# facebookresearch/brainmagick

Measured on AMD Instinct MI355X. Metric: segments/s, 208-ch x 360-sample SimpleConv + ClipLoss training step, higher is better.
Workload: dtype f32 (fp32-accurate: operands split into 2 scaled f16 planes, 3 MFMA products, fp32 accumulate; same parity tolerances as exact fp32, see DESIGN.md §2); 1 GPU; cfg2: gwilliams2022-shaped MEG C=208 T=360, F=120 features, 27 subjects, clip_conv SimpleConv (8985590 params) + ClipLoss + Adam; batch_per_gpu=256, global_batch=256, negatives=local, parallelism=dp1, comm=none, rccl_world=1, candidate_gather=none, distinct_batches=8

## Files before the change

brainmagick_amd/csrc/bm_common.h:

```cpp
#pragma once
#include <hip/hip_runtime.h>
#include <stdint.h>
#include <stdio.h>
#include <math.h>

typedef float f32x16 __attribute__((ext_vector_type(16)));
typedef float f32x4 __attribute__((ext_vector_type(4)));

#define BM_OK 0
#define BM_ERR_ARG 1001
#define BM_ERR_WORKSPACE 1002
#define BM_ERR_UNSUPPORTED 1003

extern thread_local char bm_err_buf[512];
int bm_set_error(int code, const char* fmt, ...);
int bm_check_launch(const char* what);

#define BM_REQUIRE(cond, ...)                                   \
    do {                                                        \
        if (!(cond)) return bm_set_error(BM_ERR_ARG, __VA_ARGS__); \
    } while (0)

static inline int cdiv(long a, long b) { return (int)((a + b - 1) / b); }
static inline bool prefer_big(int n) { return (long)cdiv(n, 128) * 128 <= (long)cdiv(n, 64) * 64; }
// ... 16 lines not shown
#else
    const unsigned t = (unsigned)(((unsigned long long)n * f.mul) >> 32);
#endif
    return f.shift == 0 ? n : (t + ((n - t) >> 1)) >> (f.shift - 1);
}
__host__ __device__ __forceinline__ int bm_floordiv(int a, int b) { return a >= 0 ? a / b : -((-a + b - 1) / b); }

#define BM_BKC 16
#define BM_WAVE 64

__device__ __forceinline__ int bm_xcd_remap(int id, int n) {
    const int q = n >> 3, r = n & 7;
    const int xcd = id & 7, slot = id >> 3;
    const int base = (xcd < r) ? xcd * (q + 1) : r * (q + 1) + (xcd - r) * q;
    return base + slot;
}

enum { BM_ACT_NONE = 0, BM_ACT_GELU = 1, BM_ACT_RELU = 2, BM_ACT_LEAKY = 3 };

__device__ __forceinline__ float bm_erff(float a) { return erff(a); }

__device__ __forceinline__ float bm_act(float z, int act, float leak) {
    if (act == BM_ACT_GELU) return 0.5f * z * (1.0f + bm_erff(z * 0.70710678118654752440f));
    if (act == BM_ACT_RELU) return !(z <= 0.f) ? z : 0.f;
    if (act == BM_ACT_LEAKY) return z > 0.f ? z : z * leak;
    return z;
}

__device__ __forceinline__ float bm_gelu_grad_fast(float z) {
    const float a = fabsf(z);
// ... 88 lines not shown
```

brainmagick_amd/csrc/core.hip:

```cpp
#include "bm_block.h"
#include <stdarg.h>
#include <stdlib.h>

thread_local char bm_err_buf[512] = {0};

int bm_set_error(int code, const char* fmt, ...) {
    va_list ap;
    va_start(ap, fmt);
    vsnprintf(bm_err_buf, sizeof(bm_err_buf), fmt, ap);
    va_end(ap);
    return code;
}

int bm_check_launch(const char* what) {
    hipError_t e = hipGetLastError();
    if (e != hipSuccess) return bm_set_error((int)e, "%s: launch failed: %s", what, hipGetErrorString(e));
    return BM_OK;
}

extern "C" const char* bm_last_error(void) { return bm_err_buf; }
extern "C" int bm_version(void) { return 117; }

extern "C" int bm_device_count(void) {
    int n = 0;
    hipError_t e = hipGetDeviceCount(&n);
    if (e != hipSuccess) { bm_set_error((int)e, "hipGetDeviceCount: %s", hipGetErrorString(e)); return -1; }
    return n;
}

#define FIN_THREADS 1024
#define FIN_WAVES (FIN_THREADS / 64)
__global__ __launch_bounds__(FIN_THREADS) void amax_finalize_kernel(const float* __restrict__ ws, int n,
                                                                    float* __restrict__ out) {
    __shared__ float sh[FIN_WAVES];
    bm_amax_fold<FIN_WAVES>(ws, n, out, sh);
}
// ... 38 lines not shown
```

brainmagick_amd/csrc/gemm_nt_h2w.hip:

```cpp
#include <cstdlib>
#include "gemm_nt_common.h"

typedef _Float16 f16x8 __attribute__((ext_vector_type(8)));
typedef _Float16 f16x4 __attribute__((ext_vector_type(4)));
typedef unsigned int u32x2 __attribute__((ext_vector_type(2)));

#define HG_K 32
#define HG_XQ (64 + 2)

struct GemmNTArgsH {
    const float* a; long a_sstride; long a_rstride;
    const float* x; long x_sstride; long x_rstride;
    const float* a_amax; const float* x_amax;
    const float* a_row_amax;
    float* part;
    int S, M, Cn, T, dil, nsplit;
    int tiles_m, tiles_c;
    const int* order; const int* seg;
};

__device__ __forceinline__ u32x4 hg_ld128(__amdgpu_buffer_rsrc_t rs, int voff, int soff) {
    return __builtin_amdgcn_raw_buffer_load_b128(rs, voff, soff, 0);
}
__device__ __forceinline__ unsigned hg_ld32(__amdgpu_buffer_rsrc_t rs, int voff) {
// ... 47 lines not shown
    else
        asm volatile("" :: "v"(r[0]), "v"(r[1]), "v"(r[2]), "v"(r[3]), "v"(r[4]), "v"(r[5]), "v"(r[6]), "v"(r[7]),
                     "v"(r[8]), "v"(r[9]), "v"(r[10]), "v"(r[11]));
}

#ifdef HG_TRACE
__device__ long long hg_trace_buf[64 * 4 * 8];
#define HG_T(I_) { __builtin_amdgcn_sched_barrier(0); tr[I_] = __builtin_readcyclecounter(); __builtin_amdgcn_sched_barrier(0); }
extern "C" int bm_debug_trace_read(long long* out) {
    return (int)hipMemcpyFromSymbol(out, HIP_SYMBOL(hg_trace_buf), sizeof(long long) * 64 * 4 * 8);
}
#else
#define HG_T(I_)
#endif

template <int KS, int MW, int NS, bool RS = false, bool TS = false, bool FL = false>
__global__ __launch_bounds__(256, 1) void gemm_nt_h2w_kernel(GemmNTArgsH a) {
    static_assert(!FL || RS, "the flat walk relies on the row-scaled A path (pieces inside or outside a row)");
    static_assert((MW == 5 && NS == 3) || (MW == 4 && NS == 2) || (MW == 4 && NS == 4),
                  "tile variants: 320 x 192, 256 x 128, 256 x 256");
    static_assert(!TS || (KS == 1 && !RS), "the transposed partial tile is the score contraction's");
    static_assert(KS == 1 || NS == 3, "3 taps use the 3 slots");
    constexpr int NA = 2 * MW;
    constexpr int NX = 2 * NS;
    constexpr int NP = NA + NX;
    constexpr int BM = 64 * MW;
    constexpr int BC = KS == 3 ? 64 : 64 * NS;
    constexpr int AQ = BM + 2;
    constexpr int ASLOTS = 4 * AQ;
    constexpr int PLANE = ASLOTS + NS * 4 * HG_XQ;
    constexpr int BUF = 2 * PLANE;
    constexpr int TN = MW * NS;
    constexpr int NXS = KS == 3 ? 3 : 1;
#ifdef HG_TRACE
    const long long t_kernel0 = __builtin_readcyclecounter();
    long long t_loop0 = t_kernel0, t_loop1 = t_kernel0;
#endif
    extern __shared__ __attribute__((aligned(16))) float smem[];
    u32x4* lds = reinterpret_cast<u32x4*>(smem);
    const int tid = threadIdx.x;
    const int lane = tid & 63;
    const int wave = __builtin_amdgcn_readfirstlane(tid >> 6);
    const int wm = wave >> 1, wc = wave & 1;
    const int nl = lane & 31, h = lane >> 5;

    int id = bm_xcd_remap(blockIdx.x, gridDim.x);
    const int tm = id % a.tiles_m; id /= a.tiles_m;
    const int tc = id % a.tiles_c; id /= a.tiles_c;
    const int split = id % a.nsplit;
    const int grp = id / a.nsplit;
    const int m0 = tm * BM, c0 = tc * BC;
    const int s_first = a.seg ? a.seg[grp] : 0;
    const int s_count = a.seg ? a.seg[grp + 1] - s_first : a.S;
#define HG_SEG(K_) (a.order ? a.order[s_first + (K_)] : s_first + (K_))

    const int cps = (a.T + HG_K - 1) / HG_K;
    const long nchunks = FL ? ((long)a.S * a.T + HG_K - 1) / HG_K : (long)s_count * cps;
    const long q_begin = nchunks * split / a.nsplit;
    const long q_end = nchunks * (split + 1) / a.nsplit;
    const int nst = (int)(q_end - q_begin);
    const int halo = KS == 3 ? a.dil : 0;
// ... 319 lines not shown
                }
            }
        }
    }
#ifdef HG_TRACE
    asm volatile("s_waitcnt vmcnt(0)" ::: "memory");
    if (blockIdx.x < 64 && lane == 0) {
        long long* o = hg_trace_buf + (blockIdx.x * 4 + wave) * 8;
        o[2] = t_loop0 - t_kernel0;
        o[3] = t_loop1 - t_loop0;
        o[6] = (long long)__builtin_readcyclecounter() - t_loop1;
    }
#endif
}

static int hg_family(int S, int G, int M, int Cn, int T, int KS, int dil, bool ordered) {
    if (KS != 3 && KS != 1) return 0;
    if ((G != 1 || ordered) && KS != 1) return 0;
    if (dil < 1 || dil > 32 || T < 2 * HG_K) return 0;
    if ((long)S * ((T + HG_K - 1) / HG_K) < 32L * G) return 0;
    const long work = (long)M * Cn;
    const long pad53 = (long)cdiv(M, 320) * 320 * cdiv(Cn, KS == 3 ? 64 : 192) * (KS == 3 ? 64 : 192);
    if (KS == 3) return pad53 * 4 <= work * 5 ? 1 : 0;
    const long pad42 = (long)cdiv(M, 256) * 256 * cdiv(Cn, 128) * 128;
    if (pad42 < pad53 && pad42 <= work * 2) return 2;
    return pad53 <= work * 2 ? 1 : 0;
}

extern "C" int bm_gemm_nt_h2_covers(int M, int Cn, int KS, int S, int T, int G, int dil, int ordered) {
    return hg_family(S, G, M, Cn, T, KS, dil, ordered != 0) ? 1 : 0;
// ... 1 lines not shown

extern "C" int bm_gemm_nt_h2_suggest_splits(int M, int Cn, int KS, int S, int T) {
    return bm_gemm_nt_h2_suggest_splits_grouped(M, Cn, KS, S, T, 1);
}
extern "C" int bm_gemm_nt_h2_suggest_splits_grouped(int M, int Cn, int KS, int S, int T, int G) {
    if (G < 1) G = 1;
    const int fam = hg_family(S, G, M, Cn, T, KS, 1, G > 1);
    const int tiles = (fam == 2 ? cdiv(M, 256) * cdiv(Cn, 128) : cdiv(M, 320) * cdiv(Cn, KS == 3 ? 64 : 192)) * G;
    const long chunks = (long)(S / G > 0 ? S / G : 1) * ((T + HG_K - 1) / HG_K);
    long want = 256 / tiles;
    if (want > chunks / 8) want = chunks / 8;
    if (want < 1) want = 1;
    return (int)want;
}

template <int KS, int MW, int NS, bool RS = false, bool TS = false, bool FL = false>
static int launch_gemm_nt_h2w(GemmNTArgsH g, hipStream_t stream, int ngroups = 1) {
    constexpr int PLANE = 4 * (64 * MW + 2) + NS * 4 * HG_XQ;
    const size_t lds = (size_t)2 * 2 * PLANE * 16;
    static bool attr_set = false;
    if (!attr_set) {
        hipError_t e = hipFuncSetAttribute(reinterpret_cast<const void*>(gemm_nt_h2w_kernel<KS, MW, NS, RS, TS, FL>),
                                           hipFuncAttributeMaxDynamicSharedMemorySize, (int)lds);
        if (e != hipSuccess) return bm_set_error((int)e, "gemm_nt_h2w: hipFuncSetAttribute: %s", hipGetErrorString(e));
        attr_set = true;
    }
    g.tiles_m = cdiv(g.M, 64 * MW);
    g.tiles_c = cdiv(g.Cn, KS == 3 ? 64 : 64 * NS);
    const long nblocks = (long)g.tiles_m * g.tiles_c * g.nsplit * ngroups;
    hipLaunchKernelGGL((gemm_nt_h2w_kernel<KS, MW, NS, RS, TS, FL>), dim3((unsigned)nblocks), dim3(256), lds, stream, g);
    return bm_check_launch("gemm_nt_h2w");
}

static int gemm_nt_h2_impl(const float* a, long a_sstride, long a_rstride, const float* a_amax, const float* a_row_amax,
                           const float* x, long x_sstride, long x_rstride, const float* x_amax, float* part, int S,
                           int M, int Cn, int T, int KS, int dil, int nsplit, void* stream,
                           const int* order = nullptr, const int* seg = nullptr, int G = 1) {
    BM_REQUIRE(a && x && part && a_amax && x_amax, "gemm_nt_h2: null pointer");
    BM_REQUIRE(M > 0 && Cn > 0 && T > 0 && nsplit > 0 && S >= 0, "gemm_nt_h2: bad dims");
    BM_REQUIRE(G >= 1 && (G == 1 || seg), "gemm_nt_h2: a grouped call needs seg[]");
    const bool grouped = seg != nullptr || order != nullptr;
    const int fam = hg_family(S, G, M, Cn, T, KS, dil, grouped);
    BM_REQUIRE(fam != 0, "gemm_nt_h2: shape not covered (M=%d Cn=%d T=%d KS=%d dil=%d)", M, Cn, T, KS, dil);
    if (((long)(M - 1) * a_rstride + T) * 4 >= 0x7f000000L || ((long)(Cn - 1) * x_rstride + T) * 4 >= 0x7f000000L)
        return bm_gemm_nt_x3(a, a_sstride, a_rstride, x, x_sstride, x_rstride, order, seg, part, S, G, M, Cn, T,
                             KS, dil, nsplit, stream);
    GemmNTArgsH g;
    g.a = a; g.a_sstride = a_sstride; g.a_rstride = a_rstride; g.a_amax = a_amax;
    g.x = x; g.x_sstride = x_sstride; g.x_rstride = x_rstride; g.x_amax = x_amax;
    g.a_row_amax = a_row_amax;
    g.part = part; g.S = S; g.M = M; g.Cn = Cn; g.T = T; g.dil = dil; g.nsplit = nsplit;
    g.order = order; g.seg = seg;
    hipStream_t s = (hipStream_t)stream;
    if (grouped) {
        if (fam == 2) return launch_gemm_nt_h2w<1, 4, 2>(g, s, G);
        return launch_gemm_nt_h2w<1, 5, 3>(g, s, G);
    }
    const bool rs = a_row_amax && fam == 1 && T % 4 == 0 && a_rstride % 4 == 0 && a_sstride % 4 == 0;
    const bool flat = rs && KS == 3 && T % HG_K != 0 && T >= 2 * HG_K && S > 1 &&
                      ((long)(S - 1) * a_sstride + (long)(M - 1) * a_rstride + T) * 4 < 0x7f000000L &&
                      ((long)(S - 1) * x_sstride + (long)(Cn - 1) * x_rstride + T) * 4 < 0x7f000000L &&
                      a_sstride >= T && x_sstride >= T && x_sstride % 4 == 0;
    if (flat) return launch_gemm_nt_h2w<3, 5, 3, true, false, true>(g, s);
    if (KS == 3) return rs ? launch_gemm_nt_h2w<3, 5, 3, true>(g, s) : launch_gemm_nt_h2w<3, 5, 3>(g, s);
    if (fam == 2) return launch_gemm_nt_h2w<1, 4, 2>(g, s);
    return rs ? launch_gemm_nt_h2w<1, 5, 3, true>(g, s) : launch_gemm_nt_h2w<1, 5, 3>(g, s);
}

extern "C" int bm_gemm_nt_h2(const float* a, long a_sstride, long a_rstride, const float* a_amax, const float* x,
                             long x_sstride, long x_rstride, const float* x_amax, float* part, int S, int M, int Cn,
                             int T, int KS, int dil, int nsplit, void* stream) {
    return gemm_nt_h2_impl(a, a_sstride, a_rstride, a_amax, nullptr, x, x_sstride, x_rstride, x_amax, part, S, M, Cn, T,
                           KS, dil, nsplit, stream);
}

extern "C" int bm_gemm_nt_h2_rows(const float* a, long a_sstride, long a_rstride, const float* a_amax,
                                  const float* a_row_amax, const float* x, long x_sstride, long x_rstride,
                                  const float* x_amax, float* part, int S, int M, int Cn, int T, int KS, int dil,
                                  int nsplit, void* stream) {
    return gemm_nt_h2_impl(a, a_sstride, a_rstride, a_amax, a_row_amax, x, x_sstride, x_rstride, x_amax, part, S, M, Cn,
                           T, KS, dil, nsplit, stream);
// ... 48 lines not shown
```

brainmagick_amd/csrc/pack.hip:

```cpp
#include "bm_common.h"

__global__ void pack_weights_kernel(const float* __restrict__ src, float* __restrict__ dst, int G,
                                    int M, int Cin, int KS, long sg, long sm, long sc, long sj,
                                    int flip, int Mpad, int nchunk, const float* alpha_ptr) {
    const long total = (long)G * nchunk * KS * BM_BKC * Mpad;
    const float alpha = alpha_ptr ? *alpha_ptr : 1.f;
    for (long i = (long)blockIdx.x * blockDim.x + threadIdx.x; i < total;
         i += (long)gridDim.x * blockDim.x) {
        long r = i;
        const int m = (int)(r % Mpad); r /= Mpad;
        const int cc = (int)(r % BM_BKC); r /= BM_BKC;
        const int j = (int)(r % KS); r /= KS;
        const int chunk = (int)(r % nchunk);
        const int g = (int)(r / nchunk);
        const int c = chunk * BM_BKC + cc;
        float v = 0.f;
        if (m < M && c < Cin) {
            const int jj = flip ? KS - 1 - j : j;
            v = alpha * src[g * sg + m * sm + c * sc + jj * sj];
        }
        dst[i] = v;
    }
}

// ... 78 lines not shown
        if (err) atomicExch(err, 1);
        v = 0;
    }
    out[i] = (int)v;
}

extern "C" int bm_index_to_i32(const long* idx, int B, int G, int* out, int* err_flag, void* stream) {
    BM_REQUIRE((idx && out) || B == 0, "index_to_i32: null pointer");
    BM_REQUIRE(B >= 0 && G > 0, "index_to_i32: bad dims B=%d G=%d", B, G);
    if (B == 0) return BM_OK;
    hipLaunchKernelGGL(index_to_i32_kernel, dim3((B + 255) / 256), dim3(256), 0, (hipStream_t)stream, idx, B,
                       G, out, err_flag);
    return bm_check_launch("index_to_i32");
}

__global__ void reduce_splits_kernel(const float* __restrict__ part, float* __restrict__ out, int G,
                                     int nsplit, int M, int Cn, int KS, long sg, long sm, long sc,
                                     long sj) {
    const long N = (long)Cn * KS;
    const long per = (long)M * N;
    const long total = (long)G * per;
    for (long i = (long)blockIdx.x * blockDim.x + threadIdx.x; i < total;
         i += (long)gridDim.x * blockDim.x) {
        const int g = (int)(i / per);
        const long r = i - (long)g * per;
        const int m = (int)(r / N);
        const int n = (int)(r - (long)m * N);
        const int c = n / KS, j = n - c * KS;
        const float* p = part + (long)g * nsplit * per + r;
        float s = 0.f;
        for (int k = 0; k < nsplit; ++k) s += p[(long)k * per];
        out[g * sg + m * sm + c * sc + j * sj] = s;
    }
}

__global__ void reduce_splits_vec4_kernel(const float* __restrict__ part, float* __restrict__ out, int G,
                                          int nsplit, int M, int Cn, int KS, long sg, long sm, long sc,
                                          long sj) {
    const long N = (long)Cn * KS;
    const long per = (long)M * N;
    const long total4 = (long)G * per / 4;
    for (long i4 = (long)blockIdx.x * blockDim.x + threadIdx.x; i4 < total4;
         i4 += (long)gridDim.x * blockDim.x) {
        const long i = i4 * 4;
        const int g = (int)(i / per);
        const long r = i - (long)g * per;
        const float* p = part + (long)g * nsplit * per + r;
        float4 s = make_float4(0.f, 0.f, 0.f, 0.f);
        int k = 0;
        for (; k + 8 <= nsplit; k += 8) {
            float4 v[8];
#pragma unroll
            for (int u = 0; u < 8; ++u) v[u] = *reinterpret_cast<const float4*>(p + (long)(k + u) * per);
#pragma unroll
            for (int u = 0; u < 8; ++u) { s.x += v[u].x; s.y += v[u].y; s.z += v[u].z; s.w += v[u].w; }
        }
        for (; k < nsplit; ++k) {
            const float4 v = *reinterpret_cast<const float4*>(p + (long)k * per);
            s.x += v.x; s.y += v.y; s.z += v.z; s.w += v.w;
        }
        const float sv[4] = {s.x, s.y, s.z, s.w};
#pragma unroll
        for (int e = 0; e < 4; ++e) {
            const long re = r + e;
            const int m = (int)(re / N);
            const int n = (int)(re - (long)m * N);
            const int c = n / KS, j = n - c * KS;
            out[g * sg + m * sm + c * sc + j * sj] = sv[e];
        }
    }
}

extern "C" int bm_reduce_splits(const float* part, float* out, int G, int nsplit, int M, int Cn,
                                int KS, long sg, long sm, long sc, long sj, void* stream) {
    BM_REQUIRE(part && out, "reduce_splits: null pointer");
    const long total = (long)G * M * Cn * KS;
    if (total <= 0) return BM_OK;
    const long per = (long)M * Cn * KS;
    if (per % 4 == 0 && ((uintptr_t)part % 16) == 0) {
        const long t4 = total / 4;
        const int blocks = (int)((t4 + 255) / 256 > 8192 ? 8192 : (t4 + 255) / 256);
        hipLaunchKernelGGL(reduce_splits_vec4_kernel, dim3(blocks), dim3(256), 0, (hipStream_t)stream, part,
                           out, G, nsplit, M, Cn, KS, sg, sm, sc, sj);
        return bm_check_launch("reduce_splits");
    }
    const int blocks = (int)((total + 255) / 256 > 8192 ? 8192 : (total + 255) / 256);
    hipLaunchKernelGGL(reduce_splits_kernel, dim3(blocks), dim3(256), 0, (hipStream_t)stream, part,
                       out, G, nsplit, M, Cn, KS, sg, sm, sc, sj);
    return bm_check_launch("reduce_splits");
}

__global__ void sum_over_batch_kernel(const float* __restrict__ x, float* __restrict__ out, int B,
                                      long n) {
    for (long i = (long)blockIdx.x * blockDim.x + threadIdx.x; i < n;
         i += (long)gridDim.x * blockDim.x) {
        float s = 0.f;
        for (int b = 0; b < B; ++b) s += x[(long)b * n + i];
        out[i] = s;
    }
}

extern "C" int bm_sum_over_batch(const float* x, float* out, int B, long n, void* stream) {
    BM_REQUIRE(x && out, "sum_over_batch: null pointer");
    if (n <= 0) return BM_OK;
// ... 6 lines not shown
```

brainmagick_amd/csrc/pack_h2.hip:

```cpp
#include "conv_h2_common.h"

extern "C" long bm_packed_weight_bytes_h2(int G, int M, int Cin, int KS) {
    const long mpad = bm_conv_h2_mpad(M);
    return (long)G * cdiv(Cin, 32) * KS * 2 * 4 * mpad * 8 * 2 + (long)G * mpad * 4;
}

struct PackH2Job {
    const float* src;
    unsigned short* dst;
    float* wscale;
    const float* alpha;
    long sg, sm, sc, sj;
    int M, Cin, KS, flip, Mpad, nchunk;
    int block0, nblocks;
};

#define PACK_ROWS 4

__device__ __forceinline__ void pack_h2_rows(const PackH2Job& jb, int block, float* tile, float* rs) {
    const float* __restrict__ src = jb.src;
    const int M = jb.M, Cin = jb.Cin, KS = jb.KS, Mpad = jb.Mpad, nchunk = jb.nchunk, flip = jb.flip;
    const long sg = jb.sg, sm = jb.sm, sc = jb.sc, sj = jb.sj;
    const int rows_per_group = Mpad / PACK_ROWS;
    const int g = block / rows_per_group, m0 = (block - g * rows_per_group) * PACK_ROWS;
// ... 52 lines not shown
        }
        const long stage = ((long)g * nchunk + chunk) * KS + j;
        unsigned short* out = jb.dst + stage * 2 * plane_stride + ((long)kg * Mpad + m0 + r) * 8;
        *reinterpret_cast<uint4*>(out) = *reinterpret_cast<const uint4*>(hi);
        *reinterpret_cast<uint4*>(out + plane_stride) = *reinterpret_cast<const uint4*>(lo);
    }
}

__global__ __launch_bounds__(256) void pack_weights_h2_kernel(PackH2Job jb) {
    extern __shared__ float pack_smem[];
    pack_h2_rows(jb, blockIdx.x, pack_smem + PACK_ROWS, pack_smem);
}

__global__ __launch_bounds__(256) void pack_weights_h2_batch_kernel(const PackH2Job* __restrict__ jobs, int njobs) {
    extern __shared__ float pack_smem[];
    int lo = 0, hi = njobs - 1;
    while (lo < hi) {
        const int mid = (lo + hi + 1) >> 1;
        if (jobs[mid].block0 <= (int)blockIdx.x) lo = mid; else hi = mid - 1;
    }
    const PackH2Job jb = jobs[lo];
    pack_h2_rows(jb, blockIdx.x - jb.block0, pack_smem + PACK_ROWS, pack_smem);
}

static int pack_h2_fill(PackH2Job& jb, const float* src, void* dst, int G, int M, int Cin, int KS, long sg, long sm,
                        long sc, long sj, int flip, const float* alpha_ptr) {
    BM_REQUIRE(src && dst, "pack_weights_h2: null pointer");
    BM_REQUIRE(G > 0 && M > 0 && Cin > 0 && KS > 0, "pack_weights_h2: bad dims");
    jb.Mpad = bm_conv_h2_mpad(M);
    jb.nchunk = cdiv(Cin, 32);
    const long f16_elems = (long)G * jb.nchunk * KS * 2 * 4 * jb.Mpad * 8;
    jb.src = src; jb.dst = (unsigned short*)dst;
    jb.wscale = reinterpret_cast<float*>(reinterpret_cast<char*>(dst) + f16_elems * 2);
    jb.alpha = alpha_ptr;
    jb.sg = sg; jb.sm = sm; jb.sc = sc; jb.sj = sj;
    jb.M = M; jb.Cin = Cin; jb.KS = KS; jb.flip = flip;
// ... 78 lines not shown
```

brainmagick_amd/functional.py:

```python

import torch

from . import hip_ops as H



ACT_CODES = {"none": H.ACT_NONE, "gelu": H.ACT_GELU, "relu": H.ACT_RELU, "leaky": H.ACT_LEAKY}


def _c(t: torch.Tensor) -> torch.Tensor:
    return t if t.is_contiguous() else t.contiguous()


_arange_cache = {}


def _arange_i32(n: int, device, repeat: int = 1) -> torch.Tensor:
    key = (n, repeat, device.type, device.index)
    t = _arange_cache.get(key)
    if t is None:
        if len(_arange_cache) > 64:
            _arange_cache.clear()
        t = torch.arange(n, dtype=torch.int32, device=device)
        if repeat != 1:
# ... 1 lines not shown
        if device.type == "cuda":
            torch.cuda.current_stream(device).synchronize()
        _arange_cache[key] = t
    return t


def _conv_weight_grads(dy, x, weight, KS, dil, transposed_weight):
    dst = H.grad_destination(weight)
    B, M, T = dy.shape
    Cin = x.shape[1]
    if transposed_weight:
        out = dst if dst is not None else torch.empty(weight.shape, device=dy.device, dtype=torch.float32)
        H.gemm_nt(x, dy, B, Cin, M, T, 1, 1, out=out.view(1, Cin, M, 1))
        return out.view(weight.shape) if dst is not None else out
    if dst is not None:
        H.gemm_nt(dy, x, B, M, Cin, T, KS, dil, out=dst.view(1, M, Cin, KS))
        return dst.view(weight.shape)
    return H.gemm_nt(dy, x, B, M, Cin, T, KS, dil).view(weight.shape)


def _layer_forward(x, weight, geom, res=None, **kw):
    dil, transposed, stride, pad = geom
    if pad is not None:
        assert res is None, "the strided family has no fused residual"
        KS = weight.shape[2]
        M = weight.shape[1] if transposed else weight.shape[0]
        Tout = H.conv_out_len(x.shape[2], KS, stride, dil, pad, transposed)
        wp = H.pack_strided_rows_second(weight) if transposed else H.pack_strided_rows_first(weight)
        return H.conv_strided(x, wp, M, Tout, KS, stride, dil, pad, transposed, **kw)
    assert stride == 1
    if transposed:
# ... 527 lines not shown
```

brainmagick_amd/hip_ops.py:

```python
import ctypes
import math
import typing as tp

import numpy as np
import torch

from ._lib import lib, check, BmHipError

ACT_NONE, ACT_GELU, ACT_RELU, ACT_LEAKY = 0, 1, 2, 3
BKC = 16

import os as _os
DEFAULT_COMPUTE_DTYPE = "f16x2"
COMPUTE_DTYPES = ("f32", "f32x3", "f16x2")
_compute_dtype = _os.environ.get("BM_COMPUTE_DTYPE", DEFAULT_COMPUTE_DTYPE)
if _compute_dtype not in COMPUTE_DTYPES:
    raise ValueError(f"BM_COMPUTE_DTYPE must be one of {COMPUTE_DTYPES}, got {_compute_dtype!r}")


def set_compute_dtype(name: str):
    global _compute_dtype
    if name not in COMPUTE_DTYPES:
        raise ValueError(f"compute dtype must be one of {COMPUTE_DTYPES}, got {name!r}")
    _compute_dtype = name
# ... 573 lines not shown
class _DirectArmed:
    depth = 0

    @property
    def on(self):
        return self.depth > 0


_direct_armed = _DirectArmed()


class direct_grads_armed:

    def __enter__(self):
        _direct_armed.depth += 1
        return self

    def __exit__(self, *exc):
        _direct_armed.depth -= 1
        return False


def grad_destination(param: torch.Tensor) -> tp.Optional[torch.Tensor]:
    dst = getattr(param, "_bm_grad_dst", None)
    if dst is None or dst[1][0] or param.grad is not None or not _direct_armed.on:
        return None
    dst[1][0] = True
    return dst[0]


def gemm_nt_partials(a, x, S, M, Cn, T, a_strides, x_strides, nsplit=None):
    _req(a, "gemm_nt.a")
    _req(x, "gemm_nt.x")
    family, _, nsplit = _nt_plan(M, Cn, 1, S, T, 1, 1, False, a_strides, x_strides, nsplit, partials=True)
    part = torch.empty(nsplit, M, Cn, device=a.device, dtype=torch.float32)
    _nt_launch(family, "clip_scores:gemm_nt{}", a, x, part, S, 1, M, Cn, T, 1, 1, a_strides, x_strides, None, None, nsplit)
    return part


def sum_over_batch(x: torch.Tensor) -> torch.Tensor:
    _req(x, "sum_over_batch.x")
    B = x.shape[0]
    out = torch.empty(x.shape[1:], device=x.device, dtype=torch.float32)
# ... 1324 lines not shown
```

include/bm_hip.h:

```cpp
#ifndef BM_HIP_H
#define BM_HIP_H
#ifdef __cplusplus
extern "C" {
#endif

#define BM_ACT_NONE 0
#define BM_ACT_GELU 1
#define BM_ACT_RELU 2
#define BM_ACT_LEAKY 3

int bm_version(void);
const char* bm_last_error(void);
int bm_device_count(void);

int bm_conv_mt_for(int M);
int bm_conv_mpad(int M);
int bm_conv_stats_tiles(int B, int T);
long bm_packed_weight_elems(int G, int M, int Cin, int KS);
int bm_pack_weights(const float* src, float* dst, int G, int M, int Cin, int KS, long sg, long sm,
                    long sc, long sj, int flip, const float* alpha_ptr, void* stream);
int bm_group_by_index(const long* idx, int B, int G, int* order, int* seg, int* err_flag, void* stream);
int bm_index_to_i32(const long* idx, int B, int G, int* out, int* err_flag, void* stream);
int bm_reduce_splits(const float* part, float* out, int G, int nsplit, int M, int Cn, int KS, long sg,
                     long sm, long sc, long sj, void* stream);
int bm_sum_over_batch(const float* x, float* out, int B, long n, void* stream);

int bm_conv1d_nn(const float* x, long x_bstride, const float* wpacked, const int* widx,
                 const float* bias, long bias_gstride, const float* ep_scale, const float* ep_shift, const float* res,
                 long res_bstride, float* y_pre, float* y_out, long y_bstride, float* stats, int B,
                 int Cin, int M, int T, int KS, int dil, int act, float leak, void* stream);

int bm_conv1d_out_len(int T, int KS, int stride, int dil, int pad, int transposed);
int bm_conv_strided_stats_tiles(int B, int Tout, int stride, int transposed);
int bm_conv1d_strided(const float* x, long x_bstride, const float* wpacked, const float* bias,
                      const float* ep_scale, const float* ep_shift, float* y_pre, float* y_out, long y_bstride,
                      float* stats, int B, int Cin, int M, int T, int Tout, int KS, int stride, int dil, int pad,
                      int act, float leak, void* stream);
int bm_conv1d_transposed(const float* x, long x_bstride, const float* wpacked, const float* bias,
                         const float* ep_scale, const float* ep_shift, float* y_pre, float* y_out, long y_bstride,
// ... 40 lines not shown
int bm_conv_h2_stats_tiles(int B, int T);
int bm_conv1d_nn_h2(const float* x, long x_bstride, const float* x_amax, const void* wpacked, const int* widx,
                    const float* bias, long bias_gstride, const float* ep_scale, const float* ep_shift, const float* res,
                    long res_bstride, float* y_pre, float* y_out, long y_bstride, float* stats, int B, int Cin,
                    int M, int T, int KS, int dil, int act, float leak, int G, float* y_amax_out, float* amax_ws,
                    void* stream);

int bm_gemm_nt_h2_covers(int M, int Cn, int KS, int S, int T, int G, int dil, int ordered);
int bm_gemm_nt_h2_suggest_splits(int M, int Cn, int KS, int S, int T);
int bm_gemm_nt_h2(const float* a, long a_sstride, long a_rstride, const float* a_amax, const float* x,
                  long x_sstride, long x_rstride, const float* x_amax, float* part, int S, int M, int Cn, int T,
                  int KS, int dil, int nsplit, void* stream);
int bm_gemm_nt_h2_rows(const float* a, long a_sstride, long a_rstride, const float* a_amax, const float* a_row_amax,
                       const float* x, long x_sstride, long x_rstride, const float* x_amax, float* part, int S,
                       int M, int Cn, int T, int KS, int dil, int nsplit, void* stream);

int bm_gemm_nt_h2_grouped(const float* a, long a_sstride, long a_rstride, const float* a_amax, const float* x,
                          long x_sstride, long x_rstride, const float* x_amax, const int* order, const int* seg,
                          float* part, int S, int G, int M, int Cn, int T, int nsplit, void* stream);
int bm_gemm_nt_h2_suggest_splits_grouped(int M, int Cn, int KS, int S, int T, int G);

int bm_clip_scores_h2_covers(int B, int Bc, long K);
int bm_clip_scores_h2_suggest_splits(int B, int Bc, long K);
int bm_clip_scores_h2(const float* est, const float* est_amax, const float* cand, const float* cand_amax, float* part,
                      int B, int Bc, long K, int nsplit, void* stream);

int bm_gemm_nt_suggest_splits(int M, int Cn, int KS, int S, int T, int G);
int bm_clip_suggest_splits(int M, int Cn, int S, int T);
int bm_gemm_nt(const float* a, long a_sstride, long a_rstride, const float* x, long x_sstride,
               long x_rstride, const int* order, const int* seg, float* part, int S, int G, int M,
// ... 190 lines not shown
```

Measured before the change: 17240 segments/s.

## Batch per-layer weight-gradient GEMMs into one grouped launch during backward

Result: no change. 17390 segments/s (median of 6 runs) (+0.8%).

```diff
diff --git a/brainmagick_amd/csrc/bm_common.h b/brainmagick_amd/csrc/bm_common.h
--- a/brainmagick_amd/csrc/bm_common.h
+++ b/brainmagick_amd/csrc/bm_common.h
@@ -54,6 +54,16 @@
     const int xcd = id & 7, slot = id >> 3;
     const int base = (xcd < r) ? xcd * (q + 1) : r * (q + 1) + (xcd - r) * q;
     return base + slot;
+}
+
+template <class Job>
+__device__ __forceinline__ int bm_find_job(const Job* __restrict__ jobs, int njobs, int block) {
+    int lo = 0, hi = njobs - 1;
+    while (lo < hi) {
+        const int mid = (lo + hi + 1) >> 1;
+        if (jobs[mid].block0 <= block) lo = mid; else hi = mid - 1;
+    }
+    return lo;
 }
 
 enum { BM_ACT_NONE = 0, BM_ACT_GELU = 1, BM_ACT_RELU = 2, BM_ACT_LEAKY = 3 };
diff --git a/brainmagick_amd/csrc/core.hip b/brainmagick_amd/csrc/core.hip
--- a/brainmagick_amd/csrc/core.hip
+++ b/brainmagick_amd/csrc/core.hip
@@ -19,7 +19,7 @@
 }
 
 extern "C" const char* bm_last_error(void) { return bm_err_buf; }
-extern "C" int bm_version(void) { return 117; }
+extern "C" int bm_version(void) { return 118; }
 
 extern "C" int bm_device_count(void) {
     int n = 0;
diff --git a/brainmagick_amd/csrc/gemm_nt_h2w.hip b/brainmagick_amd/csrc/gemm_nt_h2w.hip
--- a/brainmagick_amd/csrc/gemm_nt_h2w.hip
+++ b/brainmagick_amd/csrc/gemm_nt_h2w.hip
@@ -1,4 +1,5 @@
 #include <cstdlib>
+#include <cstring>
 #include "gemm_nt_common.h"
 
 typedef _Float16 f16x8 __attribute__((ext_vector_type(8)));
@@ -85,8 +86,8 @@
 #define HG_T(I_)
 #endif
 
-template <int KS, int MW, int NS, bool RS = false, bool TS = false, bool FL = false>
-__global__ __launch_bounds__(256, 1) void gemm_nt_h2w_kernel(GemmNTArgsH a) {
+template <int KS, int MW, int NS, bool RS, bool TS, bool FL>
+__device__ __forceinline__ void gemm_nt_h2w_body(const GemmNTArgsH& a, int block, int nblocks) {
     static_assert(!FL || RS, "the flat walk relies on the row-scaled A path (pieces inside or outside a row)");
     static_assert((MW == 5 && NS == 3) || (MW == 4 && NS == 2) || (MW == 4 && NS == 4),
                   "tile variants: 320 x 192, 256 x 128, 256 x 256");
@@ -115,7 +116,7 @@
     const int wm = wave >> 1, wc = wave & 1;
     const int nl = lane & 31, h = lane >> 5;
 
-    int id = bm_xcd_remap(blockIdx.x, gridDim.x);
+    int id = bm_xcd_remap(block, nblocks);
     const int tm = id % a.tiles_m; id /= a.tiles_m;
     const int tc = id % a.tiles_c; id /= a.tiles_c;
     const int split = id % a.nsplit;
@@ -465,6 +466,22 @@
 #endif
 }
 
+template <int KS, int MW, int NS, bool RS = false, bool TS = false, bool FL = false>
+__global__ __launch_bounds__(256, 1) void gemm_nt_h2w_kernel(GemmNTArgsH a) {
+    gemm_nt_h2w_body<KS, MW, NS, RS, TS, FL>(a, blockIdx.x, gridDim.x);
+}
+
+struct GemmNTJobH {
+    GemmNTArgsH args;
+    int block0, nblocks;
+};
+
+__global__ __launch_bounds__(256, 1) void gemm_nt_h2w_batch_kernel(const GemmNTJobH* __restrict__ jobs, int njobs) {
+    const int j = bm_find_job(jobs, njobs, (int)blockIdx.x);
+    const GemmNTArgsH a = jobs[j].args;
+    gemm_nt_h2w_body<3, 5, 3, true, false, true>(a, (int)blockIdx.x - jobs[j].block0, jobs[j].nblocks);
+}
+
 static int hg_family(int S, int G, int M, int Cn, int T, int KS, int dil, bool ordered) {
     if (KS != 3 && KS != 1) return 0;
     if ((G != 1 || ordered) && KS != 1) return 0;
@@ -496,10 +513,12 @@
     return (int)want;
 }
 
+template <int MW, int NS>
+static constexpr size_t hg_lds_bytes() { return (size_t)2 * 2 * (4 * (64 * MW + 2) + NS * 4 * HG_XQ) * 16; }
+
 template <int KS, int MW, int NS, bool RS = false, bool TS = false, bool FL = false>
 static int launch_gemm_nt_h2w(GemmNTArgsH g, hipStream_t stream, int ngroups = 1) {
-    constexpr int PLANE = 4 * (64 * MW + 2) + NS * 4 * HG_XQ;
-    const size_t lds = (size_t)2 * 2 * PLANE * 16;
+    const size_t lds = hg_lds_bytes<MW, NS>();
     static bool attr_set = false;
     if (!attr_set) {
         hipError_t e = hipFuncSetAttribute(reinterpret_cast<const void*>(gemm_nt_h2w_kernel<KS, MW, NS, RS, TS, FL>),
@@ -514,39 +533,134 @@
     return bm_check_launch("gemm_nt_h2w");
 }
 
-static int gemm_nt_h2_impl(const float* a, long a_sstride, long a_rstride, const float* a_amax, const float* a_row_amax,
-                           const float* x, long x_sstride, long x_rstride, const float* x_amax, float* part, int S,
-                           int M, int Cn, int T, int KS, int dil, int nsplit, void* stream,
-                           const int* order = nullptr, const int* seg = nullptr, int G = 1) {
+enum HgVariant {
+    HG_V_X3,
+    HG_V_GROUPED_42, HG_V_GROUPED_53, HG_V_FLAT, HG_V_3_ROWS, HG_V_3, HG_V_1_42, HG_V_1_ROWS, HG_V_1
+};
+
+static int hg_plan(GemmNTArgsH& g, HgVariant& variant, const float* a, long a_sstride, long a_rstride,
+                   const float* a_amax, const float* a_row_amax, const float* x, long x_sstride, long x_rstride,
+                   const float* x_amax, float* part, int S, int M, int Cn, int T, int KS, int dil, int nsplit,
+                   const int* order, const int* seg, int G) {
     BM_REQUIRE(a && x && part && a_amax && x_amax, "gemm_nt_h2: null pointer");
     BM_REQUIRE(M > 0 && Cn > 0 && T > 0 && nsplit > 0 && S >= 0, "gemm_nt_h2: bad dims");
     BM_REQUIRE(G >= 1 && (G == 1 || seg), "gemm_nt_h2: a grouped call needs seg[]");
     const bool grouped = seg != nullptr || order != nullptr;
     const int fam = hg_family(S, G, M, Cn, T, KS, dil, grouped);
     BM_REQUIRE(fam != 0, "gemm_nt_h2: shape not covered (M=%d Cn=%d T=%d KS=%d dil=%d)", M, Cn, T, KS, dil);
-    if (((long)(M - 1) * a_rstride + T) * 4 >= 0x7f000000L || ((long)(Cn - 1) * x_rstride + T) * 4 >= 0x7f000000L)
-        return bm_gemm_nt_x3(a, a_sstride, a_rstride, x, x_sstride, x_rstride, order, seg, part, S, G, M, Cn, T,
-                             KS, dil, nsplit, stream);
-    GemmNTArgsH g;
+    if (((long)(M - 1) * a_rstride + T) * 4 >= 0x7f000000L || ((long)(Cn - 1) * x_rstride + T) * 4 >= 0x7f000000L) {
+        variant = HG_V_X3;
+        return BM_OK;
+    }
     g.a = a; g.a_sstride = a_sstride; g.a_rstride = a_rstride; g.a_amax = a_amax;
     g.x = x; g.x_sstride = x_sstride; g.x_rstride = x_rstride; g.x_amax = x_amax;
     g.a_row_amax = a_row_amax;
     g.part = part; g.S = S; g.M = M; g.Cn = Cn; g.T = T; g.dil = dil; g.nsplit = nsplit;
     g.order = order; g.seg = seg;
-    hipStream_t s = (hipStream_t)stream;
     if (grouped) {
-        if (fam == 2) return launch_gemm_nt_h2w<1, 4, 2>(g, s, G);
-        return launch_gemm_nt_h2w<1, 5, 3>(g, s, G);
+        variant = fam == 2 ? HG_V_GROUPED_42 : HG_V_GROUPED_53;
+        return BM_OK;
     }
     const bool rs = a_row_amax && fam == 1 && T % 4 == 0 && a_rstride % 4 == 0 && a_sstride % 4 == 0;
     const bool flat = rs && KS == 3 && T % HG_K != 0 && T >= 2 * HG_K && S > 1 &&
                       ((long)(S - 1) * a_sstride + (long)(M - 1) * a_rstride + T) * 4 < 0x7f000000L &&
                       ((long)(S - 1) * x_sstride + (long)(Cn - 1) * x_rstride + T) * 4 < 0x7f000000L &&
                       a_sstride >= T && x_sstride >= T && x_sstride % 4 == 0;
-    if (flat) return launch_gemm_nt_h2w<3, 5, 3, true, false, true>(g, s);
-    if (KS == 3) return rs ? launch_gemm_nt_h2w<3, 5, 3, true>(g, s) : launch_gemm_nt_h2w<3, 5, 3>(g, s);
-    if (fam == 2) return launch_gemm_nt_h2w<1, 4, 2>(g, s);
-    return rs ? launch_gemm_nt_h2w<1, 5, 3, true>(g, s) : launch_gemm_nt_h2w<1, 5, 3>(g, s);
+    if (flat) variant = HG_V_FLAT;
+    else if (KS == 3) variant = rs ? HG_V_3_ROWS : HG_V_3;
+    else if (fam == 2) variant = HG_V_1_42;
+    else variant = rs ? HG_V_1_ROWS : HG_V_1;
+    return BM_OK;
+}
+
+static int gemm_nt_h2_impl(const float* a, long a_sstride, long a_rstride, const float* a_amax, const float* a_row_amax,
+                           const float* x, long x_sstride, long x_rstride, const float* x_amax, float* part, int S,
+                           int M, int Cn, int T, int KS, int dil, int nsplit, void* stream,
+                           const int* order = nullptr, const int* seg = nullptr, int G = 1) {
+    GemmNTArgsH g;
+    HgVariant variant;
+    if (int rc = hg_plan(g, variant, a, a_sstride, a_rstride, a_amax, a_row_amax, x, x_sstride, x_rstride, x_amax, part,
+                         S, M, Cn, T, KS, dil, nsplit, order, seg, G))
+        return rc;
+    hipStream_t s = (hipStream_t)stream;
+    switch (variant) {
+    case HG_V_X3:
+        return bm_gemm_nt_x3(a, a_sstride, a_rstride, x, x_sstride, x_rstride, order, seg, part, S, G, M, Cn, T,
+                             KS, dil, nsplit, stream);
+    case HG_V_GROUPED_42: return launch_gemm_nt_h2w<1, 4, 2>(g, s, G);
+    case HG_V_GROUPED_53: return launch_gemm_nt_h2w<1, 5, 3>(g, s, G);
+    case HG_V_FLAT: return launch_gemm_nt_h2w<3, 5, 3, true, false, true>(g, s);
+    case HG_V_3_ROWS: return launch_gemm_nt_h2w<3, 5, 3, true>(g, s);
+    case HG_V_3: return launch_gemm_nt_h2w<3, 5, 3>(g, s);
+    case HG_V_1_42: return launch_gemm_nt_h2w<1, 4, 2>(g, s);
+    case HG_V_1_ROWS: return launch_gemm_nt_h2w<1, 5, 3, true>(g, s);
+    default: return launch_gemm_nt_h2w<1, 5, 3>(g, s);
+    }
+}
+
+extern "C" int bm_gemm_nt_h2_job_bytes() { return (int)sizeof(GemmNTJobH); }
+
+extern "C" int bm_gemm_nt_h2_batch_covers(const float* a_row_amax, long a_sstride, long a_rstride, long x_sstride,
+                                          long x_rstride, int S, int M, int Cn, int T, int KS, int dil) {
+    GemmNTArgsH g;
+    HgVariant variant;
+    float any = 0.f;
+    if (S < 0 || M <= 0 || Cn <= 0 || T <= 0 || !hg_family(S, 1, M, Cn, T, KS, dil, false)) return 0;
+    if (hg_plan(g, variant, &any, a_sstride, a_rstride, &any, a_row_amax, &any, x_sstride, x_rstride, &any, &any, S,
+                M, Cn, T, KS, dil, 1, nullptr, nullptr, 1))
+        return 0;
+    return variant == HG_V_FLAT ? 1 : 0;
+}
+
+extern "C" int bm_gemm_nt_h2_rows_job_fill(void* job, const float* a, long a_sstride, long a_rstride,
+                                           const float* a_amax, const float* a_row_amax, const float* x,
+                                           long x_sstride, long x_rstride, const float* x_amax, float* part, int S,
+                                           int M, int Cn, int T, int KS, int dil, int nsplit, int block0) {
+    if (!job || block0 < 0) return -bm_set_error(BM_ERR_ARG, "gemm_nt_h2_rows_job_fill: bad job / block0");
+    GemmNTJobH jb;
+    HgVariant variant;
+    if (int rc = hg_plan(jb.args, variant, a, a_sstride, a_rstride, a_amax, a_row_amax, x, x_sstride, x_rstride, x_amax,
+                         part, S, M, Cn, T, KS, dil, nsplit, nullptr, nullptr, 1))
+        return -rc;
+    if (variant != HG_V_FLAT)
+        return -bm_set_error(BM_ERR_UNSUPPORTED, "gemm_nt_h2_rows_job_fill: not a flat row-scaled 3-tap contraction "
+                             "(M=%d Cn=%d T=%d KS=%d dil=%d)", M, Cn, T, KS, dil);
+    jb.args.tiles_m = cdiv(M, 320);
+    jb.args.tiles_c = cdiv(Cn, 64);
+    const long nblocks = (long)jb.args.tiles_m * jb.args.tiles_c * nsplit;
+    if (nblocks + block0 > 0x7fffffffL) return -bm_set_error(BM_ERR_ARG, "gemm_nt_h2_rows_job_fill: too many workgroups");
+    jb.block0 = block0; jb.nblocks = (int)nblocks;
+    memcpy(job, &jb, sizeof(jb));
+    return jb.nblocks;
+}
+
+extern "C" int bm_gemm_nt_h2_rows_batch(const void* jobs_dev, int njobs, int total_blocks, void* stream) {
+    BM_REQUIRE(jobs_dev && njobs > 0 && total_blocks > 0, "gemm_nt_h2_rows_batch: bad arguments");
+    const size_t lds = hg_lds_bytes<5, 3>();
+    static bool attr_set = false;
+    if (!attr_set) {
+        hipError_t e = hipFuncSetAttribute(reinterpret_cast<const void*>(gemm_nt_h2w_batch_kernel),
+                                           hipFuncAttributeMaxDynamicSharedMemorySize, (int)lds);
+        if (e != hipSuccess) return bm_set_error((int)e, "gemm_nt_h2_rows_batch: hipFuncSetAttribute: %s", hipGetErrorString(e));
+        attr_set = true;
+    }
+    hipLaunchKernelGGL(gemm_nt_h2w_batch_kernel, dim3((unsigned)total_blocks), dim3(256), lds, (hipStream_t)stream,
+                       (const GemmNTJobH*)jobs_dev, njobs);
+    return bm_check_launch("gemm_nt_h2_rows_batch");
+}
+
+extern "C" int bm_gemm_nt_h2_batch_suggest_splits(int total_tiles) {
+    static int cus = 0;
+    if (cus == 0) {
+        int dev = 0, n = 0;
+        cus = (hipGetDevice(&dev) == hipSuccess &&
+               hipDeviceGetAttribute(&n, hipDeviceAttributeMultiprocessorCount, dev) == hipSuccess && n > 0) ? n : 256;
+    }
+    if (total_tiles < 1) return 1;
+    for (long R = 1;; ++R) {
+        const long n = R * cus / total_tiles;
+        if (n >= 1 && n * total_tiles * 100 >= 95 * R * cus) return (int)(n > 0x7fff ? 0x7fff : n);
+    }
 }
 
 extern "C" int bm_gemm_nt_h2(const float* a, long a_sstride, long a_rstride, const float* a_amax, const float* x,
diff --git a/brainmagick_amd/csrc/pack.hip b/brainmagick_amd/csrc/pack.hip
--- a/brainmagick_amd/csrc/pack.hip
+++ b/brainmagick_amd/csrc/pack.hip
@@ -1,3 +1,4 @@
+#include <cstring>
 #include "bm_common.h"
 
 __global__ void pack_weights_kernel(const float* __restrict__ src, float* __restrict__ dst, int G,
@@ -116,48 +117,50 @@
     return bm_check_launch("index_to_i32");
 }
 
-__global__ void reduce_splits_kernel(const float* __restrict__ part, float* __restrict__ out, int G,
-                                     int nsplit, int M, int Cn, int KS, long sg, long sm, long sc,
-                                     long sj) {
-    const long N = (long)Cn * KS;
-    const long per = (long)M * N;
-    const long total = (long)G * per;
-    for (long i = (long)blockIdx.x * blockDim.x + threadIdx.x; i < total;
-         i += (long)gridDim.x * blockDim.x) {
+struct ReduceJob {
+    const float* part; float* out;
+    int G, nsplit, M, Cn, KS;
+    long sg, sm, sc, sj;
+    int vec4;
+    int block0, nblocks;
+};
+
+__device__ __forceinline__ void reduce_splits_scalar(const ReduceJob& jb, int block, int nblocks) {
+    const long N = (long)jb.Cn * jb.KS;
+    const long per = (long)jb.M * N;
+    const long total = (long)jb.G * per;
+    for (long i = (long)block * blockDim.x + threadIdx.x; i < total; i += (long)nblocks * blockDim.x) {
         const int g = (int)(i / per);
         const long r = i - (long)g * per;
         const int m = (int)(r / N);
         const int n = (int)(r - (long)m * N);
-        const int c = n / KS, j = n - c * KS;
-        const float* p = part + (long)g * nsplit * per + r;
+        const int c = n / jb.KS, j = n - c * jb.KS;
+        const float* p = jb.part + (long)g * jb.nsplit * per + r;
         float s = 0.f;
-        for (int k = 0; k < nsplit; ++k) s += p[(long)k * per];
-        out[g * sg + m * sm + c * sc + j * sj] = s;
-    }
-}
-
-__global__ void reduce_splits_vec4_kernel(const float* __restrict__ part, float* __restrict__ out, int G,
-                                          int nsplit, int M, int Cn, int KS, long sg, long sm, long sc,
-                                          long sj) {
-    const long N = (long)Cn * KS;
-    const long per = (long)M * N;
-    const long total4 = (long)G * per / 4;
-    for (long i4 = (long)blockIdx.x * blockDim.x + threadIdx.x; i4 < total4;
-         i4 += (long)gridDim.x * blockDim.x) {
+        for (int k = 0; k < jb.nsplit; ++k) s += p[(long)k * per];
+        jb.out[g * jb.sg + m * jb.sm + c * jb.sc + j * jb.sj] = s;
+    }
+}
+
+__device__ __forceinline__ void reduce_splits_vec4(const ReduceJob& jb, int block, int nblocks) {
+    const long N = (long)jb.Cn * jb.KS;
+    const long per = (long)jb.M * N;
+    const long total4 = (long)jb.G * per / 4;
+    for (long i4 = (long)block * blockDim.x + threadIdx.x; i4 < total4; i4 += (long)nblocks * blockDim.x) {
         const long i = i4 * 4;
         const int g = (int)(i / per);
         const long r = i - (long)g * per;
-        const float* p = part + (long)g * nsplit * per + r;
+        const float* p = jb.part + (long)g * jb.nsplit * per + r;
         float4 s = make_float4(0.f, 0.f, 0.f, 0.f);
         int k = 0;
-        for (; k + 8 <= nsplit; k += 8) {
+        for (; k + 8 <= jb.nsplit; k += 8) {
             float4 v[8];
 #pragma unroll
             for (int u = 0; u < 8; ++u) v[u] = *reinterpret_cast<const float4*>(p + (long)(k + u) * per);
 #pragma unroll
             for (int u = 0; u < 8; ++u) { s.x += v[u].x; s.y += v[u].y; s.z += v[u].z; s.w += v[u].w; }
         }
-        for (; k < nsplit; ++k) {
+        for (; k < jb.nsplit; ++k) {
             const float4 v = *reinterpret_cast<const float4*>(p + (long)k * per);
             s.x += v.x; s.y += v.y; s.z += v.z; s.w += v.w;
         }
@@ -167,29 +170,64 @@
             const long re = r + e;
             const int m = (int)(re / N);
             const int n = (int)(re - (long)m * N);
-            const int c = n / KS, j = n - c * KS;
-            out[g * sg + m * sm + c * sc + j * sj] = sv[e];
-        }
-    }
+            const int c = n / jb.KS, j = n - c * jb.KS;
+            jb.out[g * jb.sg + m * jb.sm + c * jb.sc + j * jb.sj] = sv[e];
+        }
+    }
+}
+
+__global__ void reduce_splits_kernel(ReduceJob jb) { reduce_splits_scalar(jb, blockIdx.x, gridDim.x); }
+__global__ void reduce_splits_vec4_kernel(ReduceJob jb) { reduce_splits_vec4(jb, blockIdx.x, gridDim.x); }
+
+__global__ void reduce_splits_batch_kernel(const ReduceJob* __restrict__ jobs, int njobs) {
+    const ReduceJob jb = jobs[bm_find_job(jobs, njobs, (int)blockIdx.x)];
+    if (jb.vec4) reduce_splits_vec4(jb, (int)blockIdx.x - jb.block0, jb.nblocks);
+    else reduce_splits_scalar(jb, (int)blockIdx.x - jb.block0, jb.nblocks);
+}
+
+static int reduce_splits_fill(ReduceJob& jb, const float* part, float* out, int G, int nsplit, int M, int Cn, int KS,
+                              long sg, long sm, long sc, long sj) {
+    BM_REQUIRE(part && out, "reduce_splits: null pointer");
+    const long total = (long)G * M * Cn * KS;
+    jb.part = part; jb.out = out; jb.G = G; jb.nsplit = nsplit; jb.M = M; jb.Cn = Cn; jb.KS = KS;
+    jb.sg = sg; jb.sm = sm; jb.sc = sc; jb.sj = sj;
+    jb.block0 = 0; jb.nblocks = 0; jb.vec4 = 0;
+    if (total <= 0) return BM_OK;
+    const long per = (long)M * Cn * KS;
+    jb.vec4 = per % 4 == 0 && ((uintptr_t)part % 16) == 0;
+    const long items = jb.vec4 ? total / 4 : total;
+    jb.nblocks = (int)((items + 255) / 256 > 8192 ? 8192 : (items + 255) / 256);
+    return BM_OK;
 }
 
 extern "C" int bm_reduce_splits(const float* part, float* out, int G, int nsplit, int M, int Cn,
                                 int KS, long sg, long sm, long sc, long sj, void* stream) {
-    BM_REQUIRE(part && out, "reduce_splits: null pointer");
-    const long total = (long)G * M * Cn * KS;
-    if (total <= 0) return BM_OK;
-    const long per = (long)M * Cn * KS;
-    if (per % 4 == 0 && ((uintptr_t)part % 16) == 0) {
-        const long t4 = total / 4;
-        const int blocks = (int)((t4 + 255) / 256 > 8192 ? 8192 : (t4 + 255) / 256);
-        hipLaunchKernelGGL(reduce_splits_vec4_kernel, dim3(blocks), dim3(256), 0, (hipStream_t)stream, part,
-                           out, G, nsplit, M, Cn, KS, sg, sm, sc, sj);
-        return bm_check_launch("reduce_splits");
-    }
-    const int blocks = (int)((total + 255) / 256 > 8192 ? 8192 : (total + 255) / 256);
-    hipLaunchKernelGGL(reduce_splits_kernel, dim3(blocks), dim3(256), 0, (hipStream_t)stream, part,
-                       out, G, nsplit, M, Cn, KS, sg, sm, sc, sj);
+    ReduceJob jb;
+    if (int rc = reduce_splits_fill(jb, part, out, G, nsplit, M, Cn, KS, sg, sm, sc, sj)) return rc;
+    if (jb.nblocks == 0) return BM_OK;
+    if (jb.vec4) hipLaunchKernelGGL(reduce_splits_vec4_kernel, dim3(jb.nblocks), dim3(256), 0, (hipStream_t)stream, jb);
+    else hipLaunchKernelGGL(reduce_splits_kernel, dim3(jb.nblocks), dim3(256), 0, (hipStream_t)stream, jb);
     return bm_check_launch("reduce_splits");
+}
+
+extern "C" int bm_reduce_splits_job_bytes() { return (int)sizeof(ReduceJob); }
+
+extern "C" int bm_reduce_splits_job_fill(void* job, const float* part, float* out, int nsplit, int M, int Cn, int KS,
+                                         long sm, long sc, long sj, int block0) {
+    if (!job || block0 < 0 || nsplit < 1) return -bm_set_error(BM_ERR_ARG, "reduce_splits_job_fill: bad arguments");
+    ReduceJob jb;
+    if (int rc = reduce_splits_fill(jb, part, out, 1, nsplit, M, Cn, KS, 0, sm, sc, sj)) return -rc;
+    if (jb.nblocks == 0) return -bm_set_error(BM_ERR_ARG, "reduce_splits_job_fill: empty fold");
+    jb.block0 = block0;
+    memcpy(job, &jb, sizeof(jb));
+    return jb.nblocks;
+}
+
+extern "C" int bm_reduce_splits_batch(const void* jobs_dev, int njobs, int total_blocks, void* stream) {
+    BM_REQUIRE(jobs_dev && njobs > 0 && total_blocks > 0, "reduce_splits_batch: bad arguments");
+    hipLaunchKernelGGL(reduce_splits_batch_kernel, dim3((unsigned)total_blocks), dim3(256), 0, (hipStream_t)stream,
+                       (const ReduceJob*)jobs_dev, njobs);
+    return bm_check_launch("reduce_splits_batch");
 }
 
 __global__ void sum_over_batch_kernel(const float* __restrict__ x, float* __restrict__ out, int B,
diff --git a/brainmagick_amd/csrc/pack_h2.hip b/brainmagick_amd/csrc/pack_h2.hip
--- a/brainmagick_amd/csrc/pack_h2.hip
+++ b/brainmagick_amd/csrc/pack_h2.hip
@@ -90,12 +90,7 @@
 
 __global__ __launch_bounds__(256) void pack_weights_h2_batch_kernel(const PackH2Job* __restrict__ jobs, int njobs) {
     extern __shared__ float pack_smem[];
-    int lo = 0, hi = njobs - 1;
-    while (lo < hi) {
-        const int mid = (lo + hi + 1) >> 1;
-        if (jobs[mid].block0 <= (int)blockIdx.x) lo = mid; else hi = mid - 1;
-    }
-    const PackH2Job jb = jobs[lo];
+    const PackH2Job jb = jobs[bm_find_job(jobs, njobs, (int)blockIdx.x)];
     pack_h2_rows(jb, blockIdx.x - jb.block0, pack_smem + PACK_ROWS, pack_smem);
 }
 
diff --git a/brainmagick_amd/functional.py b/brainmagick_amd/functional.py
--- a/brainmagick_amd/functional.py
+++ b/brainmagick_amd/functional.py
@@ -39,7 +39,7 @@
         H.gemm_nt(x, dy, B, Cin, M, T, 1, 1, out=out.view(1, Cin, M, 1))
         return out.view(weight.shape) if dst is not None else out
     if dst is not None:
-        H.gemm_nt(dy, x, B, M, Cin, T, KS, dil, out=dst.view(1, M, Cin, KS))
+        H.gemm_nt_into_bucket(dy, x, B, M, Cin, T, KS, dil, dst)
         return dst.view(weight.shape)
     return H.gemm_nt(dy, x, B, M, Cin, T, KS, dil).view(weight.shape)
 
diff --git a/brainmagick_amd/hip_ops.py b/brainmagick_amd/hip_ops.py
--- a/brainmagick_amd/hip_ops.py
+++ b/brainmagick_amd/hip_ops.py
@@ -611,10 +611,17 @@
 
     def __enter__(self):
         _direct_armed.depth += 1
+        if _direct_armed.depth == 1:
+            _wgrad_queue.open = True
         return self
 
-    def __exit__(self, *exc):
+    def __exit__(self, exc_type, *exc):
         _direct_armed.depth -= 1
+        try:
+            _wgrad_queue.flush(singly=exc_type is not None)
+        finally:
+            if exc_type is not None or _direct_armed.depth == 0:
+                _wgrad_queue.open = False
         return False
 
 
@@ -624,6 +631,129 @@
         return None
     dst[1][0] = True
     return dst[0]
+
+
+WGRAD_QUEUE_BYTE_CAP = 12 << 30
+_batched_wgrad = _os.environ.get("BM_BATCHED_WGRAD", "1") == "1"
+wgrad_batch_launches = 0
+
+
+def set_batched_wgrad(on: bool):
+    global _batched_wgrad
+    _batched_wgrad = bool(on)
+
+
+def get_batched_wgrad() -> bool:
+    return _batched_wgrad
+
+
+class _WgradQueue:
+    MAX_TABLES = 16
+
+    def __init__(self):
+        self.open = False
+        self.jobs: tp.List[dict] = []
+        self.held = 0
+        self.stream = None
+        self.tables: tp.Dict[tuple, tuple] = {}
+
+    def accepts(self, a, x, rows, S, M, Cn, T, KS, dil) -> bool:
+        if not (_batched_wgrad and self.open and _direct_armed.on and KS == 3 and rows is not None):
+            return False
+        if self.jobs and self.stream != torch.cuda.current_stream(a.device):
+            return False
+        family, swapped, _ = _nt_plan(M, Cn, KS, S, T, 1, dil, False, (M * T, T), (Cn * T, T))
+        return family == "h2_rows" and not swapped and \
+            bool(lib().bm_gemm_nt_h2_batch_covers(_p(rows), M * T, T, Cn * T, T, S, M, Cn, T, KS, dil))
+
+    def push(self, a, x, rows, S, M, Cn, T, dil, out) -> bool:
+        if not self.jobs:
+            try:
+                torch.autograd.Variable._execution_engine.queue_callback(self.flush)
+            except RuntimeError:
+                return False
+            self.stream = torch.cuda.current_stream(a.device)
+        self.jobs.append(dict(a=a, x=x, a_amax=amax(a), x_amax=amax(x), rows=rows, out=out, dims=(S, M, Cn, T, dil)))
+        self.held += 4 * (a.numel() + x.numel())
+        if self.held > WGRAD_QUEUE_BYTE_CAP:
+            self.flush()
+        return True
+
+    def flush(self, singly: bool = False):
+        jobs, self.jobs, self.held = self.jobs, [], 0
+        if not jobs:
+            return
+        with torch.cuda.stream(self.stream):
+            if singly or len(jobs) == 1:
+                for j in jobs:
+                    S, M, Cn, T, dil = j["dims"]
+                    gemm_nt(j["a"], j["x"], S, M, Cn, T, 3, dil, out=j["out"])
+            else:
+                self._launch(jobs)
+
+    def _launch(self, jobs):
+        global wgrad_batch_launches
+        L = lib()
+        device = jobs[0]["a"].device
+        tiles = sum(-(-j["dims"][1] // 320) * -(-j["dims"][2] // 64) for j in jobs)
+        stages = min(-(-j["dims"][0] * j["dims"][3] // 32) for j in jobs)
+        n = max(1, min(L.bm_gemm_nt_h2_batch_suggest_splits(tiles), stages // 8))
+        offs, total = [], 0
+        for j in jobs:
+            offs.append(total)
+            total += (n * j["dims"][1] * j["dims"][2] * 3 + 3) // 4 * 4
+        part = torch.empty(total, device=device, dtype=torch.float32)
+        key = (n, part.data_ptr()) + tuple(
+            (j["a"].data_ptr(), j["x"].data_ptr(), j["a_amax"].data_ptr(), j["x_amax"].data_ptr(), j["rows"].data_ptr(),
+             j["out"].data_ptr()) + j["dims"] for j in jobs)
+        table = self.tables.get(key)
+        if table is None:
+            if len(self.tables) >= self.MAX_TABLES:
+                self.tables.clear()
+            nbg, nbr = L.bm_gemm_nt_h2_job_bytes(), L.bm_reduce_splits_job_bytes()
+            host = torch.empty(len(jobs) * (nbg + nbr), dtype=torch.uint8, pin_memory=True)
+            g0 = r0 = 0
+            for i, (j, off) in enumerate(zip(jobs, offs)):
+                S, M, Cn, T, dil = j["dims"]
+                p = ctypes.c_void_p(part.data_ptr() + 4 * off)
+                ng = L.bm_gemm_nt_h2_rows_job_fill(ctypes.c_void_p(host.data_ptr() + i * nbg), _p(j["a"]), M * T, T,
+                                                   _p(j["a_amax"]), _p(j["rows"]), _p(j["x"]), Cn * T, T,
+                                                   _p(j["x_amax"]), p, S, M, Cn, T, 3, dil, n, g0)
+                nr = L.bm_reduce_splits_job_fill(ctypes.c_void_p(host.data_ptr() + len(jobs) * nbg + i * nbr), p,
+                                                 _p(j["out"]), n, M, Cn, 3, Cn * 3, 3, 1, r0)
+                if ng < 0 or nr < 0:
+                    check(-min(ng, nr), "bm_gemm_nt_h2_rows_job_fill")
+                g0 += ng
+                r0 += nr
+            dev = host.to(device, non_blocking=True)
+            table = self.tables[key] = (dev, dev[len(jobs) * nbg:], g0, r0, host)
+        dev_g, dev_r, gblocks, rblocks, _ = table
+        flops = sum(2.0 * j["dims"][0] * j["dims"][3] * j["dims"][1] * j["dims"][2] * 3 for j in jobs)
+        _timed("gemm_nt_h2w_kernel<KS=3,batch>", flops,
+               lambda: check(L.bm_gemm_nt_h2_rows_batch(_p(dev_g), len(jobs), gblocks, _stream()),
+                             "bm_gemm_nt_h2_rows_batch"))
+        _timed("reduce_splits_batch", 0.0,
+               lambda: check(L.bm_reduce_splits_batch(_p(dev_r), len(jobs), rblocks, _stream()),
+                             "bm_reduce_splits_batch"))
+        for j in jobs:
+            _touched(j["out"])
+        wgrad_batch_launches += 1
+
+
+_wgrad_queue = _WgradQueue()
+
+
+def gemm_nt_into_bucket(a: torch.Tensor, x: torch.Tensor, S: int, M: int, Cn: int, T: int, KS: int, dil: int,
+                        bucket_view: torch.Tensor):
+    _req(a, "gemm_nt.a")
+    _req(x, "gemm_nt.x")
+    rows = row_amax_of(a) if _compute_dtype == "f16x2" else None
+    if rows is not None and rows.numel() != M:
+        rows = None
+    q = _wgrad_queue
+    if q.accepts(a, x, rows, S, M, Cn, T, KS, dil) and q.push(a, x, rows, S, M, Cn, T, dil, bucket_view.view(1, M, Cn, KS)):
+        return
+    gemm_nt(a, x, S, M, Cn, T, KS, dil, out=bucket_view.view(1, M, Cn, KS))
 
 
 def gemm_nt_partials(a, x, S, M, Cn, T, a_strides, x_strides, nsplit=None):
diff --git a/include/bm_hip.h b/include/bm_hip.h
--- a/include/bm_hip.h
+++ b/include/bm_hip.h
@@ -23,6 +23,10 @@
 int bm_index_to_i32(const long* idx, int B, int G, int* out, int* err_flag, void* stream);
 int bm_reduce_splits(const float* part, float* out, int G, int nsplit, int M, int Cn, int KS, long sg,
                      long sm, long sc, long sj, void* stream);
+int bm_reduce_splits_job_bytes(void);
+int bm_reduce_splits_job_fill(void* job, const float* part, float* out, int nsplit, int M, int Cn, int KS, long sm,
+                              long sc, long sj, int block0);
+int bm_reduce_splits_batch(const void* jobs_dev, int njobs, int total_blocks, void* stream);
 int bm_sum_over_batch(const float* x, float* out, int B, long n, void* stream);
 
 int bm_conv1d_nn(const float* x, long x_bstride, const float* wpacked, const int* widx,
@@ -93,6 +97,15 @@
 int bm_gemm_nt_h2_rows(const float* a, long a_sstride, long a_rstride, const float* a_amax, const float* a_row_amax,
                        const float* x, long x_sstride, long x_rstride, const float* x_amax, float* part, int S,
                        int M, int Cn, int T, int KS, int dil, int nsplit, void* stream);
+int bm_gemm_nt_h2_job_bytes(void);
+int bm_gemm_nt_h2_batch_covers(const float* a_row_amax, long a_sstride, long a_rstride, long x_sstride, long x_rstride,
+                               int S, int M, int Cn, int T, int KS, int dil);
+int bm_gemm_nt_h2_rows_job_fill(void* job, const float* a, long a_sstride, long a_rstride, const float* a_amax,
+                                const float* a_row_amax, const float* x, long x_sstride, long x_rstride,
+                                const float* x_amax, float* part, int S, int M, int Cn, int T, int KS, int dil,
+                                int nsplit, int block0);
+int bm_gemm_nt_h2_rows_batch(const void* jobs_dev, int njobs, int total_blocks, void* stream);
+int bm_gemm_nt_h2_batch_suggest_splits(int total_tiles);
 
 int bm_gemm_nt_h2_grouped(const float* a, long a_sstride, long a_rstride, const float* a_amax, const float* x,
                           long x_sstride, long x_rstride, const float* x_amax, const int* order, const int* seg,
```
